# generic-ebpf/generic-ebpf

Measured on AMD Instinct MI355X. Metric: Mpkt/s device-resident (64-insn filter, 64B pkts); achieved HBM GB/s vs peak, higher is better.
Workload: dtype u64; 1 GPU; c4; desc=64-insn classify + array-map lookup, 64 B packets, packets_total=67108864, packets_per_gpu=67108864, packet_bytes=64, prog_slots=553, dprog_entries=122, variant=0, exec=compiled, kernel_layout=staged64, parallelism=dp1, launch=eager, faulted_packets=0

## Files before the change

### generic-ebpf_amd/csrc/asm/gen_interp.py

```python
#!/usr/bin/env python3
import os
import re
import sys

NREG = 11
_NT = int(os.environ.get("EBPF_ASM_NT", "3"))
ST_POLICY = " nt" if _NT & 1 else ""
LD_POLICY = " nt" if _NT & 2 else ""
PROBE_POLICY = ""
for _v, _n in (("EBPF_ASM_STPOL", "ST_POLICY"), ("EBPF_ASM_LDPOL", "LD_POLICY"),
               ("EBPF_ASM_PROBEPOL", "PROBE_POLICY")):
    if os.environ.get(_v):
        _p = os.environ[_v].replace("+", " ")
        globals()[_n] = "" if _p == "none" else " " + _p
PKT0 = 22
V_PKT = 38
V_LEN = 40
V_T = 41
V_STK = 42
V_L16 = 43
V_IDX = 43
V_RES = 44
H = [46, 47, 48, 49, 50, 51]
R = list(range(52, 63))
# ... 1914 lines not shown
          ".Llk_known:",
          "v_mov_b32 %s, v4" % v(H[0]), "v_mov_b32 %s, v5" % v(H[1]),
          "s_mov_b32 %s, 4" % s(S_T0), "s_mov_b32 %s, 0" % s(S_T1)] + call(".Lr_check")
    key = v(H[2])
    L += ["v_mov_b32 %s, 0" % key]
    for b in range(4):
        L += ["flat_load_ubyte %s, %s offset:%d" % (v(H[3]), vp(H[0]), b),
              "s_waitcnt vmcnt(0) lgkmcnt(0)",
              "v_lshl_or_b32 %s, %s, %d, %s" % (key, v(H[3]), 8 * b, key)]
    L += ["s_mov_b32 %s, 0" % s(S_T2),
          ".Llk_map:",
          "s_cmp_ge_u32 %s, %s" % (s(S_T2), s(S_NMAPS)),
          "s_cbranch_scc1 .Llk_done",
          "s_lshl_b32 %s, %s, 5" % (s(S_T3), s(S_T2)),
          "s_load_dwordx8 s[%d:%d], %s, %s" % (S_REC, S_REC + 7, sp(S_MAPS), s(S_T3)),
          "s_waitcnt lgkmcnt(0)",
          "v_cmp_eq_u64_e64 %s, v[2:3], s[64:65]" % sp(S_JUNK),
          "v_cmp_gt_u32_e64 vcc, s69, %s" % key,
          "s_and_b64 vcc, vcc, %s" % sp(S_JUNK),
          "v_mov_b32 %s, s68" % v(H[3]),
          "v_mad_u64_u32 %s, %s, %s, %s, s[66:67]" % (vp(H[4]), sp(S_JUNK), key, v(H[3])),
          "v_cndmask_b32 v0, v0, %s, vcc" % v(H[4]),
          "v_cndmask_b32 v1, v1, %s, vcc" % v(H[5]),
          "s_add_u32 %s, %s, 1" % (s(S_T2), s(S_T2)),
          "s_branch .Llk_map",
          ".Llk_done:",
          mode_test(MODE_JIT),
          "s_cbranch_scc1 .Llk_jit"] + dispatch(12) + [
          ".Llk_jit:",
          "s_add_u32 %s, %s, s12" % (s(S_JUNK), s(S_CB)),
          "s_addc_u32 %s, %s, 0" % (s(S_JUNK + 1), s(S_CB + 1)),
          "s_setpc_b64 %s" % sp(S_JUNK)] + [
          ".Llk_sched:"] + goto(".Lr_schedule")
    L += hlookup_routine()
    L += update_routine()
    L += hdelete_routine()
    L += vstore_routine()
    L += [".Lr_ovlfix:"] + ovl_fix("L", (H[2], H[3])) + ["s_setpc_b64 %s" % sp(S_LINK)]
    L += [".Lr_prefetch:",
          "s_mov_b64 exec, -1",
          "s_cmp_ge_u32 %s, %s" % (s(S_T0), s(S_NGROUPS)),
          "s_cbranch_scc1 .Lpf_ret",
          "s_lshl_b32 s66, %s, 6" % s(S_T0),
          "s_sub_u32 s66, %s, s66" % s(S_COUNT),
          "s_mov_b32 s64, %s" % s(S_T0),
          "s_mov_b32 s65, 0",
          "s_lshl_b64 s[64:65], s[64:65], 12",
          "s_add_u32 s64, s64, %s" % s(S_DATA),
          "s_addc_u32 s65, s65, %s" % s(S_DATA + 1),
          "s_mov_b32 s67, %s" % s(S_PKTLDS)] + dma_lane_offsets(v(H[4]), v(H[5]))
    for qq in range(4):
        L += ["s_sub_i32 s68, s66, %d" % (16 * qq),
              "s_max_i32 s68, s68, 0",
              "s_min_u32 s68, s68, 16",
              "s_lshl_b32 s68, s68, 6",
              "v_cmp_gt_u32_e64 vcc, s68, %s" % v(H[4]),
              "s_mov_b64 exec, vcc",
              "s_mov_b32 m0, s67",
              "s_nop 0",
              "global_load_lds_dwordx4 %s, s[64:65]%s" % (v(H[4]), LD_POLICY)]
        if qq < 3:
            L += ["s_add_u32 s64, s64, 1024", "s_addc_u32 s65, s65, 0",
                  "s_add_u32 s67, s67, 1024"]
    L += [".Lpf_ret:",
          "s_setpc_b64 %s" % sp(S_LINK)]
    return L


def kernel(name, staged, jit=False):
    k = "K%s%s" % ("s" if staged else "g", "j" if jit else "")
    L = [".globl %s" % name, ".p2align 8", ".type %s,@function" % name, "%s:" % name]
    if name == "ebpf_jit_s64" and phased() and SLOTS == 16:
        L += [".globl ebpf_jit_s64w", ".type ebpf_jit_s64w,@function", "ebpf_jit_s64w:"]
    L += ["v_readfirstlane_b32 %s, v0" % s(S_WAVE),
          "s_lshr_b32 %s, %s, 6" % (s(S_WAVE), s(S_WAVE)),
          "s_load_dwordx16 s[%d:%d], %s" % (S_PROG, S_PROG + 15, karg_regs(
              ("prog", S_PROG), ("maps", S_MAPS), ("data", S_DATA), ("offsets", S_OFFS),
              ("off_base", S_OFFBASE), ("ret", S_RET), ("faults", S_FAULTS), ("hist", S_HIST))),
          "s_load_dwordx8 s[%d:%d], %s" % (S_COUNT, S_COUNT + 7, karg_regs(
              ("count", S_COUNT), ("stride", S_STRIDE), ("start", S_START), ("nmaps", S_NMAPS),
              ("nentries", S_NENT), ("stack_stride", S_STKSTRIDE), ("lds_stack_base", S_LDSBASE))),
          "s_load_dword %s, %s" % (s(S_GSTRIDE), karg("total_waves")),
          "s_load_dword %s, %s" % (s(S_PKTLDS), karg("lds_pkt_base")),
          "s_mov_b64 %s, src_shared_base" % sp(S_SHARED),
          "v_mov_b32 v%d, 0x00010203" % V_SEL,
          "s_getpc_b64 %s" % sp(S_CB),
          ".L%s_pc:" % k,
          "s_add_u32 %s, %s, .Lcb-.L%s_pc" % (s(S_CB), s(S_CB), k),
          "s_addc_u32 %s, %s, 0" % (s(S_CB + 1), s(S_CB + 1)),
          "v_mbcnt_lo_u32_b32 %s, -1, 0" % v(H[0]),
          "v_mbcnt_hi_u32_b32 %s, -1, %s" % (v(H[0]), v(H[0])),
          "v_lshlrev_b32 v%d, 4, %s" % (V_L16, v(H[0])),
          "s_mov_b32 %s, -1" % s(S_PREVG),
          "s_waitcnt lgkmcnt(0)",
          "s_mov_b32 %s, %d" % (s(S_MODE), (staged << MODE_STAGED) | (jit << MODE_JIT)),
          "s_load_dword %s, %s" % (s(S_T3), karg("vflags"))] + (
          ["s_load_dword %s, %s" % (s(S_WPHASE), karg("wphase")) if staged else
           "s_mov_b32 %s, 0" % s(S_WPHASE),
           "s_mov_b32 %s, 0" % s(S_PEND)] if phased() else []) + [
          "s_waitcnt lgkmcnt(0)",
          "s_bitcmp1_b32 %s, %d" % (s(S_T3), VF_OVERLAY),
          "s_cbranch_scc0 .L%s_noovl" % k,
          mode_set(MODE_OVERLAY),
          ".L%s_noovl:" % k,
          "s_bitcmp1_b32 %s, %d" % (s(S_T3), VF_EXTENTS),
          "s_cbranch_scc0 .L%s_noext" % k,
          mode_set(MODE_EXTENTS),
          ".L%s_noext:" % k]
    if staged:
        L += ["s_bitcmp1_b32 %s, %d" % (s(S_T3), VF_KEEP),
              "s_cbranch_scc0 .L%s_nokeep" % k,
              mode_set(MODE_KEEP),
              ".L%s_nokeep:" % k]
    if not staged:
        L += ["s_bitcmp1_b32 %s, %d" % (s(S_PKTLDS), PKTLDS_HDRSTAGE),
              "s_cbranch_scc0 .L%s_nogs" % k,
              mode_set(MODE_HDRSTAGE),
              ".L%s_nogs:" % k,
              "s_bitcmp1_b32 %s, %d" % (s(S_PKTLDS), PKTLDS_HDRKEEP),
              "s_cbranch_scc0 .L%s_nohl" % k,
              mode_set(MODE_KEEP),
              ".L%s_nohl:" % k,
              "s_and_b32 %s, %s, 0x%x" % (s(S_PKTLDS), s(S_PKTLDS), (1 << PKTLDS_HDRKEEP) - 1)]
    L += ["s_branch .Lprologue"]
    return L


def lane_index(dst):
    if STAGED_IMAGE:
        return ["v_lshrrev_b32 %s, 4, v%d" % (v(dst), V_L16)]
    return ["v_mbcnt_lo_u32_b32 %s, -1, 0" % v(dst), "v_mbcnt_hi_u32_b32 %s, -1, %s" % (v(dst), v(dst))]


def lane_pkt_index(dst):
    if STAGED_IMAGE:
        return ["v_lshrrev_b32 %s, 4, v%d" % (v(dst), V_L16),
                "v_lshl_add_u32 %s, %s, 6, %s" % (v(dst), s(S_GROUP), v(dst))]
    return ["v_mov_b32 %s, v%d" % (v(dst), V_IDX)]


def pkt_setup(idx, tag):
    return ["s_mov_b64 %s, exec" % sp(S_MASK),
            "s_cmp_eq_u64 %s, 0" % sp(S_OFFS),
            "s_cbranch_scc0 .Lps_offsets_%s" % tag,
            "v_mov_b32 %s, %s" % (v(H[1]), s(S_STRIDE)),
            "v_mad_u64_u32 v[%d:%d], %s, v%d, %s, %s" % (V_PKT, V_PKT + 1, sp(S_JUNK), idx,
                                                         v(H[1]), sp(S_DATA)),
            "v_mov_b32 v%d, %s" % (V_LEN, s(S_STRIDE)),
            "s_branch .Lps_stage_%s" % tag,
            ".Lps_offsets_%s:" % tag,
            mode_test(MODE_EXTENTS),
            "s_cselect_b32 %s, 16, 8" % s(S_JUNK),
            "v_mov_b32 %s, %s" % (v(H[1]), s(S_JUNK)),
            "v_mad_u64_u32 %s, %s, v%d, %s, %s" % (vp(H[4]), sp(S_JUNK), idx, v(H[1]), sp(S_OFFS)),
            "global_load_dwordx2 %s, %s, off offset:8" % (vp(R[0]), vp(H[4])),
            "global_load_dwordx2 %s, %s, off" % (vp(H[4]), vp(H[4])),
            "s_waitcnt vmcnt(0)",
            "v_sub_co_u32 v%d, vcc, %s, %s" % (V_LEN, v(R[0]), v(H[4])),
            "v_subb_co_u32 %s, vcc, %s, %s, vcc" % (v(R[1]), v(R[1]), v(H[5])),
            "v_cmp_ne_u32_e32 vcc, 0, %s" % v(R[1]),
            "v_cndmask_b32 v%d, v%d, 0, vcc" % (V_LEN, V_LEN),
            "v_mov_b32 %s, %s" % (v(R[2]), s(S_OFFBASE + 1)),
            "v_sub_co_u32 %s, vcc, %s, %s" % (v(H[4]), v(H[4]), s(S_OFFBASE)),
            "v_subb_co_u32 %s, vcc, %s, %s, vcc" % (v(H[5]), v(H[5]), v(R[2])),
            "v_lshl_add_u64 v[%d:%d], %s, 0, %s" % (V_PKT, V_PKT + 1, vp(H[4]), sp(S_DATA)),
            ] + [
            ".Lps_stage_%s:" % tag,
            mode_test(MODE_HDRSTAGE),
            "s_cbranch_scc0 .Lps_done_%s" % tag,
            "v_cmp_lt_u32_e64 vcc, 63, v%d" % V_LEN,
            "s_and_b64 exec, %s, vcc" % sp(S_MASK),
            "s_cbranch_execz .Lps_done_%s" % tag] + [
            "global_load_dwordx4 v[%d:%d], v[%d:%d], off offset:%d" % (PKT0 + 4 * q, PKT0 + 4 * q + 3,
                                                                       V_PKT, V_PKT + 1, 16 * q)
            for q in range(4)] + [
            "s_waitcnt vmcnt(0)",
            mode_test(MODE_KEEP),
            "s_cbranch_scc0 .Lps_done_%s" % tag,
            "v_mbcnt_lo_u32_b32 %s, -1, 0" % v(H[1]),
            "v_mbcnt_hi_u32_b32 %s, -1, %s" % (v(H[1]), v(H[1])),
            "v_lshl_add_u32 %s, %s, 2, %s" % (v(H[1]), v(H[1]), s(S_PKTLDS))] + lds_pkt_dwords(v(H[1])) + [
            ".Lps_done_%s:" % tag,
            "s_mov_b64 exec, %s" % sp(S_MASK)]
# ... 91 lines not shown
                sk = ".Lph_%s%d_%d_%s" % ("r" if ragged else "f", half, j, tag)
                out += ["s_bitcmp1_b32 %s, %d" % (P, j), "s_cbranch_scc0 %s" % sk]
                if not ragged:
                    if own:
                        out += ["s_cmp_ge_u32 %s, %d" % (s(S_T3), i),
                                "s_cselect_b64 s[66:67], s[60:61], s[64:65]"]
                    out.append("global_store_dwordx2 %s, v[%d:%d], s[%d:%d] offset:%d%s" % (
                        v(R[0]), V_RB + 2 * j, V_RB + 2 * j + 1, 66 if own else 62,
                        67 if own else 63, 512 * i, ST_POLICY))
                else:
                    if own:
                        out += ["s_cmp_ge_u32 %s, %d" % (s(S_T3), i),
                                "s_cselect_b32 %s, %s, %s" % (s(S_BYTES), s(S_T1), s(S_T2))]
                    else:
                        out.append("s_mov_b32 %s, %s" % (s(S_BYTES), s(S_T0)))
                    out += ["s_add_u32 %s, %s, %d" % (s(S_BYTES), s(S_BYTES), i),
                            "s_lshl_b32 s66, %s, 6" % s(S_BYTES),
                            "s_sub_u32 s66, %s, s66" % s(S_COUNT),
                            "v_cmp_gt_u32_e64 vcc, s66, %s" % v(R[1]),
                            "s_mov_b64 exec, vcc",
                            "s_lshl_b32 s66, %s, 9" % s(S_BYTES),
                            "s_lshr_b32 s67, %s, 23" % s(S_BYTES),
                            "s_add_u32 s66, s66, %s" % s(S_RET),
                            "s_addc_u32 s67, s67, %s" % s(S_RET + 1),
                            "global_store_dwordx2 %s, v[%d:%d], s[66:67]%s" % (
                                v(R[0]), V_RB + 2 * j, V_RB + 2 * j + 1, ST_POLICY),
                            "s_mov_b64 exec, -1"]
                out.append(sk + ":")
        return out

    for ragged in (False, True):
        if ragged:
            L += [".Lph_ragged_%s:" % tag,
                  "v_lshrrev_b32 %s, 4, v%d" % (v(R[1]), V_L16)]
        if len(halves) > 1:
            L += ["s_bitcmp1_b32 %s, 31" % P,
                  "s_cbranch_scc1 .Lph_%sh1_%s" % ("r" if ragged else "f", tag)]
        L += slots_of(0, ragged) + ["s_branch .Lph_done_%s" % tag]
        if len(halves) > 1:
            L += [".Lph_%sh1_%s:" % ("r" if ragged else "f", tag)] + slots_of(1, ragged) + [
                  "s_branch .Lph_done_%s" % tag]
    L += [".Lph_done_%s:" % tag,
          "s_and_b32 %s, %s, 0x80000000" % (P, P),
          "s_branch .Lsp_none_%s" % tag,
          ".Lph_off_%s:" % tag]
    return L


def store_prev_results(tag, final):
    L = store_phased(tag, final) if phased() else []
    L += ["s_cmp_eq_u32 %s, -1" % s(S_PREVG),
         "s_cbranch_scc1 .Lsp_none_%s" % tag]
    if not final and RETK > 1:
        L += ["s_and_b32 %s, %s, %s" % (s(S_T0), s(S_PREVG), s(S_KMASK)),
              "s_cmp_lg_u32 %s, %s" % (s(S_T0), s(S_KMASK)),
              "s_cbranch_scc1 .Lsp_none_%s" % tag]
    L += ["s_mov_b64 exec, -1",
          "s_andn2_b32 %s, %s, %s" % (s(S_T0), s(S_PREVG), s(S_KMASK)) if RETK > 1 else
          "s_mov_b32 %s, %s" % (s(S_T0), s(S_PREVG)),
          ] + (["v_lshrrev_b32 %s, 4, v%d" % (v(R[1]), V_L16),
                "v_lshl_add_u32 %s, %s, 6, %s" % (v(R[1]), s(S_T0), v(R[1]))] if STAGED_IMAGE else
               ["v_mov_b32 %s, v%d" % (v(R[1]), V_IDX)]) + [
          "v_lshlrev_b32 %s, 3, %s" % (v(R[0]), v(R[1]))]
    for k in range(RETK):
        if k:
            L += ["s_cmp_lt_u32 %s, %d" % (s(S_KMASK), k),
                  "s_cbranch_scc1 .Lsp_none_%s" % tag,
                  "v_add_u32 %s, 64, %s" % (v(R[1]), v(R[1]))]
        L += ["v_cmp_gt_u32_e64 vcc, %s, %s" % (s(S_COUNT), v(R[1])),
              "s_mov_b64 exec, vcc",
              "global_store_dwordx2 %s, v[%d:%d], %s offset:%d%s" % (
                  v(R[0]), V_RB + 2 * k, V_RB + 2 * k + 1, sp(S_RET), 512 * k, ST_POLICY)]
    L.append(".Lsp_none_%s:" % tag)
    return L


def next_group(dst):
    return ["s_and_b32 %s, %s, %s" % (s(dst), s(S_GROUP), s(S_KMASK)),
            "s_cmp_eq_u32 %s, %s" % (s(dst), s(S_KMASK)),
            "s_cselect_b32 %s, %s, 1" % (s(dst), s(S_GSTRIDE)),
            "s_add_u32 %s, %s, %s" % (s(dst), s(dst), s(S_GROUP))]


def common_group_code():
    L = [".Lcb:",
         "ebpf_cb:",
         ".Lprologue:"]
    L += ["s_lshl_b32 %s, %s, 6" % (s(S_T0), s(S_WAVE)),
          "v_add_u32 %s, %s, %s" % (v(H[1]), s(S_T0), v(H[0])),
          "v_mul_lo_u32 %s, %s, %s" % (v(H[4]), v(H[1]), s(S_STKSTRIDE)),
          "v_add_u32 v%d, %s, %s" % (V_STK, s(S_LDSBASE), v(H[4]))]
    L += ["v_lshlrev_b32 %s, 2, %s" % (v(H[2]), v(H[1])),
          "v_mov_b32 %s, 0" % v(H[3]),
          "ds_write_b32 %s, %s" % (v(H[2]), v(H[3]))]
    L += ["v_lshlrev_b32 %s, 2, %s" % (v(H[4]), v(H[1])),
          "s_mov_b32 %s, 0" % s(S_T2),
          ".Lmc_loop:",
          "s_cmp_ge_u32 %s, %s" % (s(S_T2), s(S_NMAPS)),
          "s_cbranch_scc1 .Lmc_done",
          "s_lshl_b32 %s, %s, 5" % (s(S_T3), s(S_T2)),
          "s_load_dwordx8 s[%d:%d], %s, %s" % (S_REC, S_REC + 7, sp(S_MAPS), s(S_T3)),
          "s_waitcnt lgkmcnt(0)",
          "s_add_u32 %s, %s, 1" % (s(S_T2), s(S_T2)),
          "s_cmp_eq_u32 s70, -1",
          "s_cbranch_scc1 .Lmc_loop",
          "s_mul_i32 %s, s68, s69" % s(S_T1),
          "s_mov_b32 %s, 0" % s(S_T0),
          ".Lmc_chunk:",
          "s_cmp_ge_u32 %s, %s" % (s(S_T0), s(S_T1)),
          "s_cbranch_scc1 .Lmc_zero",
          "v_add_u32 %s, %s, %s" % (v(H[5]), s(S_T0), v(H[4])),
          "v_cmp_gt_u32_e64 vcc, %s, %s" % (s(S_T1), v(H[5])),
          "s_mov_b64 exec, vcc",
          "global_load_dword %s, %s, s[66:67]" % (v(H[3]), v(H[5])),
          "s_waitcnt vmcnt(0)",
          "v_add_u32 %s, s70, %s" % (v(H[5]), v(H[5])),
          "ds_write_b32 %s, %s" % (v(H[5]), v(H[3])),
          "s_mov_b64 exec, -1",
          "s_add_u32 %s, %s, 1024" % (s(S_T0), s(S_T0)),
          "s_branch .Lmc_chunk",
          ".Lmc_zero:",
          "s_bitcmp1_b32 s71, 29",
          "s_cbranch_scc0 .Lmc_loop",
          "s_and_b32 %s, s71, 0xffff" % s(S_T3),
          "v_mov_b32 %s, 0" % v(H[3]),
          "s_mov_b32 %s, 0" % s(S_T0),
          ".Lmc_zchunk:",
          "s_cmp_ge_u32 %s, %s" % (s(S_T0), s(S_T1)),
          "s_cbranch_scc1 .Lmc_loop",
          "v_add_u32 %s, %s, %s" % (v(H[5]), s(S_T0), v(H[4])),
          "v_cmp_gt_u32_e64 vcc, %s, %s" % (s(S_T1), v(H[5])),
          "s_mov_b64 exec, vcc",
          "v_add_u32 %s, %s, %s" % (v(H[5]), s(S_T3), v(H[5])),
          "ds_write_b32 %s, %s" % (v(H[5]), v(H[3])),
          "s_mov_b64 exec, -1",
          "s_add_u32 %s, %s, 1024" % (s(S_T0), s(S_T0)),
          "s_branch .Lmc_zchunk",
          ".Lmc_done:",
          "s_waitcnt lgkmcnt(0)",
          "s_barrier"]
    L += ["s_add_u32 %s, %s, 63" % (s(S_NGROUPS), s(S_COUNT)),
          "s_lshr_b32 %s, %s, 6" % (s(S_NGROUPS), s(S_NGROUPS)),
          "s_lshl_b32 %s, s2, 2" % s(S_GROUP),
          "s_add_u32 %s, %s, %s" % (s(S_GROUP), s(S_GROUP), s(S_WAVE)),
          "s_lshr_b32 %s, %s, %d" % (s(S_T1), s(S_GSTRIDE), WAVES_SB_SHIFT),
          "s_and_b32 %s, %s, 0xffff" % (s(S_GSTRIDE), s(S_GSTRIDE)),
          "s_lshl_b32 %s, 1, %s" % (s(S_KMASK), s(S_T1)),
          "s_sub_u32 %s, %s, 1" % (s(S_KMASK), s(S_KMASK)),
          "s_lshl_b32 %s, %s, %s" % (s(S_GROUP), s(S_GROUP), s(S_T1)),
          ] + [
          "s_lshl_b32 %s, %s, %s" % (s(S_GSTRIDE), s(S_GSTRIDE), s(S_T1)),
          "s_sub_u32 %s, %s, %s" % (s(S_GSTRIDE), s(S_GSTRIDE), s(S_KMASK)),
          "s_lshl_b32 %s, %s, 12" % (s(S_T0), s(S_WAVE)),
          "s_add_u32 %s, %s, %s" % (s(S_PKTLDS), s(S_PKTLDS), s(S_T0)),
          mode_test(MODE_STAGED),
          "s_cbranch_scc0 .Lgroup_check",
          "s_mov_b32 %s, %s" % (s(S_T0), s(S_GROUP))] + call(".Lr_prefetch") + [
          "s_branch .Lgroup_check"]
    L += [".Lgroup_done:"]
    L += slot_commit() + next_group(S_T0) + [
          "s_and_b32 %s, %s, 0x%x" % (s(S_BYTES), s(S_MODE), 1 << MODE_KEEP | 1 << MODE_STAGED),
          "s_cmp_eq_u32 %s, 0x4001" % s(S_BYTES),
          "s_cbranch_scc0 .Lgd_nokeep"] + call(".Lr_prefetch") + [
          ".Lgd_nokeep:",
          "s_mov_b32 %s, %s" % (s(S_GROUP), s(S_T0)),
          ".Lgroup_check:",
          "s_mov_b64 exec, -1",
          "s_cmp_lt_u32 %s, %s" % (s(S_GROUP), s(S_NGROUPS)),
          "s_cbranch_scc0 .Lfinish",
          ] + (
          ["s_cmp_eq_u32 %s, 0" % s(S_WPHASE),
           "s_cbranch_scc1 .Lgc_noclock",
           "s_memrealtime s[%d:%d]" % (S_CLOCK, S_CLOCK + 1),
           ".Lgc_noclock:"] if phased() else []) + lane_index(H[0]) + [
          "v_lshl_add_u32 v%d, %s, 6, %s" % (V_GIDX, s(S_GROUP), v(H[0])),
          "v_cmp_gt_u32_e64 %s, %s, v%d" % (sp(S_ALIVE), s(S_COUNT), V_GIDX),
          ] + [
          mode_test(MODE_STAGED),
          "s_cbranch_scc0 .Lgs_general",
          "s_waitcnt vmcnt(0)",
          "v_and_b32 %s, 0x300, v%d" % (v(H[1]), V_L16),
          "v_mad_u32_u24 %s, %s, 3, v%d" % (v(H[1]), v(H[1]), V_L16),
          "v_add_u32 %s, %s, %s" % (v(H[1]), s(S_PKTLDS), v(H[1]))]
    for q in range(4):
        L.append("ds_read_b128 v[%d:%d], %s offset:%d" % (PKT0 + 4 * q, PKT0 + 4 * q + 3,
                                                          v(H[1]), 256 * q))
    L += ["s_waitcnt lgkmcnt(0)",
          mode_test(MODE_KEEP),
          "s_cbranch_scc0 .Lgs_pf_dma",
          "v_lshrrev_b32 %s, 2, v%d" % (v(H[1]), V_L16),
          "v_add_u32 %s, %s, %s" % (v(H[1]), s(S_PKTLDS), v(H[1]))] + lds_pkt_dwords(v(H[1])) + [
          "s_branch .Lgs_pf_done",
          ".Lgs_pf_dma:"] + next_group(S_T0) + [
          "s_lshr_b32 %s, %s, 6" % (s(S_BYTES), s(S_COUNT)),
          "s_cmp_lt_u32 %s, %s" % (s(S_T0), s(S_BYTES)),
          "s_cbranch_scc0 .Lgs_pf_slow",
          "s_lshr_b32 s65, %s, 20" % s(S_T0),
          "s_lshl_b32 s64, %s, 12" % s(S_T0),
          "s_add_u32 s64, s64, %s" % s(S_DATA),
          "s_addc_u32 s65, s65, %s" % s(S_DATA + 1),
          "s_mov_b64 exec, -1"] + dma_lane_offsets(v(H[4]), v(H[5])) + [
          "s_mov_b32 m0, %s" % s(S_PKTLDS),
          "s_nop 0"] + [
          "global_load_lds_dwordx4 %s, s[64:65] offset:%d%s" % (v(H[4]), 1024 * qq, LD_POLICY)
          for qq in range(4)] + [
          "s_branch .Lgs_pf_done",
          ".Lgs_pf_slow:"] + call(".Lr_prefetch") + [
          ".Lgs_pf_done:",
          mode_test(MODE_JIT),
          "s_cbranch_scc1 .Lgs_init",
          "s_mov_b64 exec, %s" % sp(S_ALIVE),
          "v_mov_b32 %s, 64" % v(H[1]),
          "v_mad_u64_u32 v[%d:%d], %s, v%d, %s, %s" % (V_PKT, V_PKT + 1, sp(S_JUNK), V_GIDX,
                                                       v(H[1]), sp(S_DATA)),
          "v_mov_b32 v%d, 64" % V_LEN,
          "s_branch .Lgs_init",
          ".Lgs_general:",
          "s_mov_b64 exec, %s" % sp(S_ALIVE)] + pkt_setup(V_GIDX, "g") + [
          ".Lgs_init:"] + store_prev_results("g", False) + [
          "s_mov_b32 %s, %s" % (s(S_PREVG), s(S_GROUP))] + ([] if STAGED_IMAGE else [
          "s_mov_b64 exec, -1",
          "v_mov_b32 v%d, v%d" % (V_IDX, V_GIDX)]) + [
          "s_mov_b64 exec, %s" % sp(S_ALIVE),
          "s_cmp_eq_u64 %s, 0" % sp(S_FAULTS),
          "s_cbranch_scc1 .Lgs_nofz",
          ] + lane_pkt_index(R[9]) + [
          "v_mov_b32 %s, 0" % v(R[8]),
          "global_store_byte %s, %s, %s" % (v(R[9]), v(R[8]), sp(S_FAULTS)),
          ".Lgs_nofz:",
          mode_test(MODE_JIT),
          "s_cbranch_scc0 .Lgs_interp"] + goto("ebpf_jit_area+%d" % JIT_ENTRY_OFF) + [
          ".Lgs_interp:"]
    for r in range(0, 20, 2):
        if r != 2:
            L.append("v_mov_b64 v[%d:%d], 0" % (r, r + 1))
    L += ["v_mov_b64 v[2:3], v[%d:%d]" % (V_PKT, V_PKT + 1),
          "v_add_u32 v20, %s, v%d" % (s(S_STKSTRIDE), V_STK),
          "v_mov_b32 v21, %s" % s(S_SHARED + 1),
          "s_lshl_b32 %s, %s, 5" % (s(S_T0), s(S_START)),
          "v_mov_b32 v%d, %s" % (V_T, s(S_T0))] + goto(".Lr_schedule")
    HR = HIST_REPLICA_BYTES
    L += [".Lfinish:"] + store_prev_results("f", True)
    L += [".Lfinish_body:",
          "s_mov_b64 exec, -1",
          "s_waitcnt vmcnt(0) lgkmcnt(0)",
          "s_barrier"]
    L += lane_index(H[0]) + [
          "s_lshl_b32 %s, %s, 6" % (s(S_T0), s(S_WAVE)),
          "v_add_u32 %s, %s, %s" % (v(H[1]), s(S_T0), v(H[0])),
          "s_mov_b32 %s, 0" % s(S_T2),
          ".Lfd_loop:",
          "s_cmp_ge_u32 %s, %s" % (s(S_T2), s(S_NMAPS)),
          "s_cbranch_scc1 .Lfd_done",
          "s_lshl_b32 %s, %s, 5" % (s(S_T3), s(S_T2)),
          "s_load_dwordx8 s[%d:%d], %s, %s" % (S_REC, S_REC + 7, sp(S_MAPS), s(S_T3)),
          "s_waitcnt lgkmcnt(0)",
          "s_add_u32 %s, %s, 1" % (s(S_T2), s(S_T2)),
          "s_bitcmp1_b32 s71, 29",
          "s_cbranch_scc0 .Lfd_loop",
          "s_mul_i32 %s, s68, s69" % s(S_T1),
          "s_add_u32 %s, %s, 63" % (s(S_BYTES), s(S_T1)),
          "s_and_b32 %s, %s, -64" % (s(S_BYTES), s(S_BYTES)),
          "s_add_u32 s66, s66, %s" % s(S_BYTES),
          "s_addc_u32 s67, s67, 0",
          "s_and_b32 %s, s71, 0xffff" % s(S_T3),
          "s_bitcmp1_b32 s71, 28",
          "s_cselect_b32 %s, 3, 2" % s(S_CODE),
          "v_lshlrev_b32 %s, %s, %s" % (v(H[2]), s(S_CODE), v(H[1])),
          "s_lshl_b32 %s, 256, %s" % (s(S_BYTES), s(S_CODE)),
          ".Lfd_word:",
          "v_cmp_gt_u32_e64 vcc, %s, %s" % (s(S_T1), v(H[2])),
          "s_and_saveexec_b64 %s, vcc" % sp(S_MASK),
          "s_cbranch_execz .Lfd_next",
          "v_add_u32 %s, %s, %s" % (v(H[3]), s(S_T3), v(H[2])),
          "v_mov_b32 %s, 0" % v(R[3]),
          "s_cmp_eq_u32 %s, 3" % s(S_CODE),
          "s_cbranch_scc0 .Lfd_r4",
          "ds_read_b64 %s, %s" % (vp(R[2]), v(H[3])),
          "s_branch .Lfd_r",
          ".Lfd_r4:",
          "ds_read_b32 %s, %s" % (v(R[2]), v(H[3])),
          ".Lfd_r:",
          "s_waitcnt lgkmcnt(0)",
          "v_cmp_ne_u64_e64 vcc, 0, %s" % vp(R[2]),
          "s_and_b64 exec, exec, vcc",
          "s_cbranch_execz .Lfd_next",
          "v_mov_b32 %s, %s" % (v(R[0]), v(H[2])),
          "s_cmp_eq_u32 %s, 3" % s(S_CODE),
          "s_cbranch_scc0 .Lfd_w4",
          "global_atomic_add_x2 %s, %s, s[66:67]" % (v(R[0]), vp(R[2])),
          "s_branch .Lfd_next",
          ".Lfd_w4:",
          "global_atomic_add %s, %s, s[66:67]" % (v(R[0]), v(R[2])),
          ".Lfd_next:",
          "s_mov_b64 exec, %s" % sp(S_MASK),
          "v_add_u32 %s, %s, %s" % (v(H[2]), s(S_BYTES), v(H[2])),
          "v_cmp_gt_u32_e64 vcc, %s, %s" % (s(S_T1), v(H[2])),
          "s_and_b64 vcc, vcc, exec",
          "s_cbranch_scc1 .Lfd_word",
          "s_mov_b64 exec, -1",
          "s_branch .Lfd_loop",
          ".Lfd_done:",
          "s_mov_b64 exec, -1",
          "s_cmp_eq_u64 %s, 0" % sp(S_HIST),
          "s_cbranch_scc1 .Lfin_end",
          ] + lane_index(H[0]) + [
          "s_lshl_b32 %s, %s, 6" % (s(S_T0), s(S_WAVE)),
          "v_add_u32 %s, %s, %s" % (v(H[1]), s(S_T0), v(H[0])),
          "v_lshlrev_b32 %s, 2, %s" % (v(H[2]), v(H[1])),
          "ds_read_b32 %s, %s" % (v(H[3]), v(H[2])),
          "s_load_dwordx2 %s, %s" % (sp(S_REC), karg("hist_rows")),
          "s_load_dwordx4 s[68:71], %s" % karg("hist_user", "hist_flags", "nwg"),
          "s_waitcnt lgkmcnt(0)",
          "s_cmp_eq_u64 %s, 0" % sp(S_REC),
          "s_cbranch_scc1 .Lfin_atomic",
          "s_and_b32 %s, s2, 7" % s(S_T1),
          "s_mul_i32 %s, %s, %d" % (s(S_T1), s(S_T1), HR),
          "v_lshlrev_b32 %s, 3, %s" % (v(R[0]), v(H[1])),
          "v_add_u32 %s, %s, %s" % (v(R[0]), s(S_T1), v(R[0])),
          "v_mov_b32 %s, %s" % (v(R[2]), v(H[3])),
          "v_mov_b32 %s, 0" % v(R[3]),
          "v_cmp_ne_u32_e64 vcc, 0, %s" % v(H[3]),
          "s_and_saveexec_b64 %s, vcc" % sp(S_SAVE),
          "s_cbranch_execz .Lfin_noadd",
          "global_atomic_add_x2 %s, %s, %s" % (v(R[0]), vp(R[2]), sp(S_REC)),
          ".Lfin_noadd:",
          "s_mov_b64 exec, -1",
          "s_waitcnt vmcnt(0)",
          "s_barrier",
          "s_cmp_eq_u32 %s, 0" % s(S_WAVE),
          "s_cbranch_scc0 .Lfin_flag",
          "s_mov_b64 exec, 1",
          "s_and_b32 %s, s2, 7" % s(S_T1),
          "s_lshl_b32 %s, %s, 6" % (s(S_T0), s(S_T1)),
          "s_add_u32 %s, %s, %d" % (s(S_T0), s(S_T0), HIST_TICKET_OFF),
          "v_mov_b32 %s, %s" % (v(R[4]), s(S_T0)),
          "v_mov_b32 %s, 1" % v(R[5]),
          "global_atomic_add %s, %s, %s, %s sc0" % (v(R[6]), v(R[4]), v(R[5]), sp(S_REC)),
          "s_sub_u32 %s, s71, 1" % s(S_T3),
          "s_sub_u32 %s, %s, %s" % (s(S_T3), s(S_T3), s(S_T1)),
          "s_lshr_b32 %s, %s, 3" % (s(S_T3), s(S_T3)),
          "s_waitcnt vmcnt(0)",
          "v_readfirstlane_b32 %s, %s" % (s(S_T2), v(R[6])),
          "s_cmp_eq_u32 %s, %s" % (s(S_T2), s(S_T3)),
          "s_cselect_b32 %s, 1, 0" % s(S_T2),
          "s_cbranch_scc0 .Lfin_setflag",
          "v_mov_b32 %s, 0" % v(R[10]),
          "global_atomic_swap %s, %s, %s, %s sc0" % (v(R[8]), v(R[4]), v(R[10]), sp(S_REC)),
          "v_mov_b32 %s, %d" % (v(R[9]), HIST_TICKET_OFF + 64 * HIST_REPLICAS),
          "global_atomic_add %s, %s, %s, %s sc0" % (v(R[6]), v(R[9]), v(R[5]), sp(S_REC)),
          "s_min_u32 %s, s71, %d" % (s(S_T3), HIST_REPLICAS),
          "s_sub_u32 %s, %s, 1" % (s(S_T3), s(S_T3)),
          "s_waitcnt vmcnt(0)",
          "v_readfirstlane_b32 %s, %s" % (s(S_T2), v(R[6])),
          "s_cmp_eq_u32 %s, %s" % (s(S_T2), s(S_T3)),
          "s_cselect_b32 %s, 1, 0" % s(S_T2),
          ".Lfin_setflag:",
          "v_mov_b32 %s, %s" % (v(R[7]), s(S_T2)),
          "v_mov_b32 %s, 0" % v(R[8]),
          "ds_write_b32 %s, %s" % (v(R[8]), v(R[7])),
          "s_mov_b64 exec, -1",
          "s_waitcnt lgkmcnt(0)",
          ".Lfin_flag:",
          "s_barrier",
          "v_mov_b32 %s, 0" % v(R[8]),
          "ds_read_b32 %s, %s" % (v(R[7]), v(R[8])),
          "s_waitcnt lgkmcnt(0)",
          "v_readfirstlane_b32 %s, %s" % (s(S_T2), v(R[7])),
          "s_cmp_eq_u32 %s, 0" % s(S_T2),
          "s_cbranch_scc1 .Lfin_end",
          "v_lshlrev_b32 %s, 3, %s" % (v(R[0]), v(H[1])),
          "v_mov_b32 v24, 0",
          "v_mov_b32 v25, 0"]
    for r in range(HIST_REPLICAS):
        L += ["v_add_u32 v%d, %d, %s" % (16 + r, r * HR, v(R[0])),
              "global_atomic_swap_x2 v[%d:%d], v%d, v[24:25], %s sc0" % (2 * r, 2 * r + 1, 16 + r,
                                                                       sp(S_REC))]
    L += ["s_waitcnt vmcnt(0)"]
    for r in range(1, HIST_REPLICAS):
        L += ["v_lshl_add_u64 v[0:1], v[%d:%d], 0, v[0:1]" % (2 * r, 2 * r + 1)]
    L += ["s_bitcmp1_b32 s70, %d" % HIST_STORE,
          "s_cbranch_scc0 .Lfin_add",
          "global_store_dwordx2 %s, v[0:1], s[68:69]" % v(R[0]),
          "s_branch .Lfin_faults",
          ".Lfin_add:",
          "global_atomic_add_x2 %s, v[0:1], s[68:69]" % v(R[0]),
          ".Lfin_faults:",
          "s_cmp_eq_u32 %s, 0" % s(S_WAVE),
          "s_cbranch_scc0 .Lfin_end",
          "s_mov_b64 exec, 1",
          "v_mov_b32 v16, 2048",
          "global_atomic_swap_x2 v[2:3], v16, v[24:25], %s sc0" % sp(S_REC),
          "v_mov_b32 v17, %d" % (HIST_TICKET_OFF + 64 * HIST_REPLICAS),
          "global_atomic_swap v18, v17, v24, %s sc0" % sp(S_REC),
          "s_waitcnt vmcnt(0)",
          "s_bitcmp1_b32 s70, %d" % HIST_STORE,
          "s_cbranch_scc0 .Lfin_fadd",
          "global_store_dwordx2 v16, v[2:3], s[68:69]",
          "s_branch .Lfin_end",
          ".Lfin_fadd:",
          "global_atomic_add_x2 v16, v[2:3], s[68:69]",
          "s_branch .Lfin_end",
          ".Lfin_atomic:",
          "v_cmp_ne_u32_e64 vcc, 0, %s" % v(H[3]),
          "s_and_saveexec_b64 %s, vcc" % sp(S_SAVE),
          "v_lshlrev_b32 %s, 3, %s" % (v(R[0]), v(H[1])),
          "v_mov_b32 %s, %s" % (v(R[2]), v(H[3])),
          "v_mov_b32 %s, 0" % v(R[3]),
          "global_atomic_add_x2 %s, %s, %s" % (v(R[0]), vp(R[2]), sp(S_HIST)),
          ".Lfin_end:",
          "s_waitcnt vmcnt(0)",
          "s_endpgm"]
    return L


def link_kernel():
    return [".globl ebpf_asm_link", ".p2align 8", ".type ebpf_asm_link,@function",
            "ebpf_asm_link:",
            "s_load_dwordx2 s[4:5], %s" % karg("entries", table=LINK_ARGS),
            "s_load_dword s6, %s" % karg("count", table=LINK_ARGS),
            "s_getpc_b64 s[8:9]",
            ".Llink_base:",
            "s_add_u32 s10, s8, .Lhandler_table-.Llink_base",
            "s_addc_u32 s11, s9, 0",
            "v_lshl_add_u32 v1, s2, 6, v0",
            "s_waitcnt lgkmcnt(0)",
            "v_cmp_gt_u32_e64 vcc, s6, v1",
            "s_and_b64 exec, exec, vcc",
            "s_cbranch_execz .Llink_end",
            "v_mov_b32 v2, 32",
            "v_mad_u64_u32 v[2:3], s[12:13], v1, v2, s[4:5]",
            "global_load_dword v4, v[2:3], off",
            "s_waitcnt vmcnt(0)",
            "v_mov_b32 v6, 4",
            "v_mad_u64_u32 v[6:7], s[12:13], v4, v6, s[10:11]",
            "global_load_dword v8, v[6:7], off",
            "s_waitcnt vmcnt(0)",
            "v_ashrrev_i32 v9, 31, v8",
            "v_lshl_add_u64 v[10:11], v[8:9], 0, s[8:9]",
            "global_store_dwordx2 v[2:3], v[10:11], off",
            ".Llink_end:",
            "s_waitcnt vmcnt(0)",
            "s_endpgm"]


def kd(name, lds, vgprs, sgprs, kernarg, wgsize):
    return [".rodata", ".p2align 6", ".amdhsa_kernel %s" % name,
            ".amdhsa_group_segment_fixed_size %d" % lds,
            ".amdhsa_private_segment_fixed_size 0",
            ".amdhsa_kernarg_size %d" % kernarg,
            ".amdhsa_user_sgpr_count 2",
            ".amdhsa_user_sgpr_kernarg_segment_ptr 1",
            ".amdhsa_system_sgpr_workgroup_id_x 1",
            ".amdhsa_system_vgpr_workitem_id 0",
            ".amdhsa_next_free_vgpr %d" % vgprs,
            ".amdhsa_next_free_sgpr %d" % sgprs,
            ".amdhsa_accum_offset %d" % vgprs,
            ".amdhsa_reserve_vcc 1",
            ".amdhsa_reserve_xnack_mask 0",
            ".amdhsa_ieee_mode 0",
            ".amdhsa_dx10_clamp 0",
            ".end_amdhsa_kernel", ".text"]


def metadata(kernels):
    out = [".amdgpu_metadata", "---", "amdhsa.kernels:"]
    for name, kernarg, lds, vgprs, sgprs, wg in kernels:
        out += ["  - .args:",
                "      - .offset: 0",
                "        .size: %d" % kernarg,
                "        .value_kind: by_value",
                "    .group_segment_fixed_size: %d" % lds,
                "    .kernarg_segment_align: 8",
                "    .kernarg_segment_size: %d" % kernarg,
                "    .max_flat_workgroup_size: %d" % wg,
                "    .name: %s" % name,
                "    .private_segment_fixed_size: 0",
                "    .sgpr_count: %d" % sgprs,
                "    .symbol: %s.kd" % name,
                "    .vgpr_count: %d" % vgprs,
                "    .wavefront_size: 64"]
    out += ["amdhsa.target: amdgcn-amd-amdhsa--gfx950:xnack-", "amdhsa.version:", "  - 1", "  - 2",
            "...", ".end_amdgpu_metadata"]
    return out


JIT_AREA_BYTES = 512 * 1024
JIT_ENTRY_OFF = 16
ENTRY_SGPR_RE = None


def entry_reads(lines):
    import re
    global ENTRY_SGPR_RE
    if ENTRY_SGPR_RE is None:
# ... 294 lines not shown
```

Measured before the change: 84820 Mpkt/s.

## Pipeline map-cache prologue loads and overlap prologue/finish latencies

Hoists the vflags/wphase kernel-argument loads into the first scalar load batch so only one lgkmcnt wait is needed. Rewrites the map-to-LDS copy loop to issue up to 16 global loads into distinct VGPRs before a single drain, instead of waiting on each load. The LDS barrier now comes after the staged prefetch is issued, so the two overlap. The finish path drops a vmcnt wait and issues the fault-counter swaps before the histogram swaps so their latencies overlap. It uses v0-v31 as temporaries in the prologue and adds nop padding, which risks register clobbering and ordering bugs.

```diff
diff --git a/generic-ebpf_amd/csrc/asm/gen_interp.py b/generic-ebpf_amd/csrc/asm/gen_interp.py
--- a/generic-ebpf_amd/csrc/asm/gen_interp.py
+++ b/generic-ebpf_amd/csrc/asm/gen_interp.py
@@ -2020,6 +2020,8 @@
               ("nentries", S_NENT), ("stack_stride", S_STKSTRIDE), ("lds_stack_base", S_LDSBASE))),
           "s_load_dword %s, %s" % (s(S_GSTRIDE), karg("total_waves")),
           "s_load_dword %s, %s" % (s(S_PKTLDS), karg("lds_pkt_base")),
+          "s_load_dword %s, %s" % (s(S_T3), karg("vflags"))] + (
+          ["s_load_dword %s, %s" % (s(S_WPHASE), karg("wphase"))] if phased() and staged else []) + [
           "s_mov_b64 %s, src_shared_base" % sp(S_SHARED),
           "v_mov_b32 v%d, 0x00010203" % V_SEL,
           "s_getpc_b64 %s" % sp(S_CB),
@@ -2032,11 +2034,9 @@
           "s_mov_b32 %s, -1" % s(S_PREVG),
           "s_waitcnt lgkmcnt(0)",
           "s_mov_b32 %s, %d" % (s(S_MODE), (staged << MODE_STAGED) | (jit << MODE_JIT)),
-          "s_load_dword %s, %s" % (s(S_T3), karg("vflags"))] + (
-          ["s_load_dword %s, %s" % (s(S_WPHASE), karg("wphase")) if staged else
-           "s_mov_b32 %s, 0" % s(S_WPHASE),
-           "s_mov_b32 %s, 0" % s(S_PEND)] if phased() else []) + [
-          "s_waitcnt lgkmcnt(0)",
+          ] + (
+          ([] if staged else ["s_mov_b32 %s, 0" % s(S_WPHASE)]) +
+          ["s_mov_b32 %s, 0" % s(S_PEND)] if phased() else []) + [
           "s_bitcmp1_b32 %s, %d" % (s(S_T3), VF_OVERLAY),
           "s_cbranch_scc0 .L%s_noovl" % k,
           mode_set(MODE_OVERLAY),
@@ -2294,63 +2294,13 @@
             "s_add_u32 %s, %s, %s" % (s(dst), s(dst), s(S_GROUP))]
 
 
+MC_SLOTS = 16
+
+
 def common_group_code():
     L = [".Lcb:",
          "ebpf_cb:",
          ".Lprologue:"]
-    L += ["s_lshl_b32 %s, %s, 6" % (s(S_T0), s(S_WAVE)),
-          "v_add_u32 %s, %s, %s" % (v(H[1]), s(S_T0), v(H[0])),
-          "v_mul_lo_u32 %s, %s, %s" % (v(H[4]), v(H[1]), s(S_STKSTRIDE)),
-          "v_add_u32 v%d, %s, %s" % (V_STK, s(S_LDSBASE), v(H[4]))]
-    L += ["v_lshlrev_b32 %s, 2, %s" % (v(H[2]), v(H[1])),
-          "v_mov_b32 %s, 0" % v(H[3]),
-          "ds_write_b32 %s, %s" % (v(H[2]), v(H[3]))]
-    L += ["v_lshlrev_b32 %s, 2, %s" % (v(H[4]), v(H[1])),
-          "s_mov_b32 %s, 0" % s(S_T2),
-          ".Lmc_loop:",
-          "s_cmp_ge_u32 %s, %s" % (s(S_T2), s(S_NMAPS)),
-          "s_cbranch_scc1 .Lmc_done",
-          "s_lshl_b32 %s, %s, 5" % (s(S_T3), s(S_T2)),
-          "s_load_dwordx8 s[%d:%d], %s, %s" % (S_REC, S_REC + 7, sp(S_MAPS), s(S_T3)),
-          "s_waitcnt lgkmcnt(0)",
-          "s_add_u32 %s, %s, 1" % (s(S_T2), s(S_T2)),
-          "s_cmp_eq_u32 s70, -1",
-          "s_cbranch_scc1 .Lmc_loop",
-          "s_mul_i32 %s, s68, s69" % s(S_T1),
-          "s_mov_b32 %s, 0" % s(S_T0),
-          ".Lmc_chunk:",
-          "s_cmp_ge_u32 %s, %s" % (s(S_T0), s(S_T1)),
-          "s_cbranch_scc1 .Lmc_zero",
-          "v_add_u32 %s, %s, %s" % (v(H[5]), s(S_T0), v(H[4])),
-          "v_cmp_gt_u32_e64 vcc, %s, %s" % (s(S_T1), v(H[5])),
-          "s_mov_b64 exec, vcc",
-          "global_load_dword %s, %s, s[66:67]" % (v(H[3]), v(H[5])),
-          "s_waitcnt vmcnt(0)",
-          "v_add_u32 %s, s70, %s" % (v(H[5]), v(H[5])),
-          "ds_write_b32 %s, %s" % (v(H[5]), v(H[3])),
-          "s_mov_b64 exec, -1",
-          "s_add_u32 %s, %s, 1024" % (s(S_T0), s(S_T0)),
-          "s_branch .Lmc_chunk",
-          ".Lmc_zero:",
-          "s_bitcmp1_b32 s71, 29",
-          "s_cbranch_scc0 .Lmc_loop",
-          "s_and_b32 %s, s71, 0xffff" % s(S_T3),
-          "v_mov_b32 %s, 0" % v(H[3]),
-          "s_mov_b32 %s, 0" % s(S_T0),
-          ".Lmc_zchunk:",
-          "s_cmp_ge_u32 %s, %s" % (s(S_T0), s(S_T1)),
-          "s_cbranch_scc1 .Lmc_loop",
-          "v_add_u32 %s, %s, %s" % (v(H[5]), s(S_T0), v(H[4])),
-          "v_cmp_gt_u32_e64 vcc, %s, %s" % (s(S_T1), v(H[5])),
-          "s_mov_b64 exec, vcc",
-          "v_add_u32 %s, %s, %s" % (v(H[5]), s(S_T3), v(H[5])),
-          "ds_write_b32 %s, %s" % (v(H[5]), v(H[3])),
-          "s_mov_b64 exec, -1",
-          "s_add_u32 %s, %s, 1024" % (s(S_T0), s(S_T0)),
-          "s_branch .Lmc_zchunk",
-          ".Lmc_done:",
-          "s_waitcnt lgkmcnt(0)",
-          "s_barrier"]
     L += ["s_add_u32 %s, %s, 63" % (s(S_NGROUPS), s(S_COUNT)),
           "s_lshr_b32 %s, %s, 6" % (s(S_NGROUPS), s(S_NGROUPS)),
           "s_lshl_b32 %s, s2, 2" % s(S_GROUP),
@@ -2365,10 +2315,85 @@
           "s_sub_u32 %s, %s, %s" % (s(S_GSTRIDE), s(S_GSTRIDE), s(S_KMASK)),
           "s_lshl_b32 %s, %s, 12" % (s(S_T0), s(S_WAVE)),
           "s_add_u32 %s, %s, %s" % (s(S_PKTLDS), s(S_PKTLDS), s(S_T0)),
+          "s_mov_b64 exec, -1"]
+    L += ["s_lshl_b32 %s, %s, 6" % (s(S_T0), s(S_WAVE)),
+          "v_add_u32 %s, %s, %s" % (v(H[1]), s(S_T0), v(H[0])),
+          "v_mul_lo_u32 %s, %s, %s" % (v(H[4]), v(H[1]), s(S_STKSTRIDE)),
+          "v_add_u32 v%d, %s, %s" % (V_STK, s(S_LDSBASE), v(H[4]))]
+    L += ["v_lshlrev_b32 %s, 2, %s" % (v(H[2]), v(H[1])),
+          "v_mov_b32 %s, 0" % v(H[3]),
+          "ds_write_b32 %s, %s" % (v(H[2]), v(H[3]))]
+    NS = MC_SLOTS
+    L += ["v_lshlrev_b32 %s, 2, %s" % (v(H[4]), v(H[1])),
+          "s_mov_b32 %s, 0" % s(S_T2),
+          "s_mov_b32 %s, 0" % s(S_T0),
+          "s_mov_b32 %s, 0" % s(S_T1),
+          ".Lmc_s0:",
+          "s_mov_b32 %s, 0" % s(S_CODE)]
+    for k in range(NS):
+        L += [".Lmc_s%d:" % k if k else ".Lmc_s0b:",
+              "s_cmp_lt_u32 %s, %s" % (s(S_T0), s(S_T1)),
+              "s_cbranch_scc1 .Lmc_i%d" % k,
+              ".Lmc_a%d:" % k,
+              "s_cmp_ge_u32 %s, %s" % (s(S_T2), s(S_NMAPS)),
+              "s_cbranch_scc1 .Lmc_w%d" % k,
+              "s_lshl_b32 %s, %s, 5" % (s(S_T3), s(S_T2)),
+              "s_load_dwordx8 s[%d:%d], %s, %s" % (S_REC, S_REC + 7, sp(S_MAPS), s(S_T3)),
+              "s_add_u32 %s, %s, 1" % (s(S_T2), s(S_T2)),
+              "s_waitcnt lgkmcnt(0)",
+              "s_cmp_eq_u32 s70, -1",
+              "s_cbranch_scc1 .Lmc_a%d" % k,
+              "s_mul_i32 %s, s68, s69" % s(S_T1),
+              "s_mov_b32 %s, 0" % s(S_T0),
+              "s_bitcmp1_b32 s71, 29",
+              "s_cbranch_scc0 .Lmc_s%s" % (k if k else "0b")] + call(".Lmc_zero") + [
+              "s_branch .Lmc_s%s" % (k if k else "0b"),
+              ".Lmc_i%d:" % k,
+              "v_add_u32 %s, %s, %s" % (v(H[5]), s(S_T0), v(H[4])),
+              "v_cmp_gt_u32_e64 vcc, %s, %s" % (s(S_T1), v(H[5])),
+              "s_mov_b64 exec, vcc",
+              "global_load_dword v%d, %s, s[66:67]" % (k, v(H[5])),
+              "s_mov_b64 exec, -1",
+              "v_add_u32 %s, s70, %s" % (v(H[5]), v(H[5])),
+              "v_cndmask_b32 v%d, -1, %s, vcc" % (NS + k, v(H[5])),
+              "s_add_u32 %s, %s, 1024" % (s(S_T0), s(S_T0))]
+    L += ["s_mov_b32 %s, 1" % s(S_CODE)]
+    for k in range(NS, 0, -1):
+        L += [".Lmc_w%d:" % k,
+              "s_waitcnt vmcnt(0)",
+              "s_mov_b64 exec, -1",
+              "v_cmp_ne_u32_e64 vcc, -1, v%d" % (NS + k - 1),
+              "s_mov_b64 exec, vcc",
+              "ds_write_b32 v%d, v%d" % (NS + k - 1, k - 1)]
+    L += [".Lmc_w0:",
+          "s_mov_b64 exec, -1",
+          "s_cmp_eq_u32 %s, 1" % s(S_CODE),
+          "s_cbranch_scc1 .Lmc_s0",
           mode_test(MODE_STAGED),
-          "s_cbranch_scc0 .Lgroup_check",
+          "s_cbranch_scc0 .Lpro_nopf",
           "s_mov_b32 %s, %s" % (s(S_T0), s(S_GROUP))] + call(".Lr_prefetch") + [
-          "s_branch .Lgroup_check"]
+          ".Lpro_nopf:",
+          "s_waitcnt lgkmcnt(0)",
+          "s_barrier",
+          "s_branch .Lgroup_check",
+          ".Lmc_zero:",
+          "s_and_b32 %s, s71, 0xffff" % s(S_T3),
+          "v_mov_b32 %s, 0" % v(H[3]),
+          "s_mov_b32 %s, 0" % s(S_BYTES),
+          ".Lmc_zchunk:",
+          "s_cmp_ge_u32 %s, %s" % (s(S_BYTES), s(S_T1)),
+          "s_cbranch_scc1 .Lmc_zret",
+          "v_add_u32 %s, %s, %s" % (v(H[5]), s(S_BYTES), v(H[4])),
+          "v_cmp_gt_u32_e64 vcc, %s, %s" % (s(S_T1), v(H[5])),
+          "s_mov_b64 exec, vcc",
+          "v_add_u32 %s, %s, %s" % (v(H[5]), s(S_T3), v(H[5])),
+          "ds_write_b32 %s, %s" % (v(H[5]), v(H[3])),
+          "s_mov_b64 exec, -1",
+          "s_add_u32 %s, %s, 1024" % (s(S_BYTES), s(S_BYTES)),
+          "s_branch .Lmc_zchunk",
+          ".Lmc_zret:",
+          "s_setpc_b64 %s" % sp(S_LINK)]
+    L += ["s_nop 0"] * 5
     L += [".Lgroup_done:"]
     L += slot_commit() + next_group(S_T0) + [
           "s_and_b32 %s, %s, 0x%x" % (s(S_BYTES), s(S_MODE), 1 << MODE_KEEP | 1 << MODE_STAGED),
@@ -2455,7 +2480,7 @@
     L += [".Lfinish:"] + store_prev_results("f", True)
     L += [".Lfinish_body:",
           "s_mov_b64 exec, -1",
-          "s_waitcnt vmcnt(0) lgkmcnt(0)",
+          "s_waitcnt lgkmcnt(0)",
           "s_barrier"]
     L += lane_index(H[0]) + [
           "s_lshl_b32 %s, %s, 6" % (s(S_T0), s(S_WAVE)),
@@ -2583,7 +2608,16 @@
           "s_cbranch_scc1 .Lfin_end",
           "v_lshlrev_b32 %s, 3, %s" % (v(R[0]), v(H[1])),
           "v_mov_b32 v24, 0",
-          "v_mov_b32 v25, 0"]
+          "v_mov_b32 v25, 0",
+          "s_cmp_eq_u32 %s, 0" % s(S_WAVE),
+          "s_cbranch_scc0 .Lfin_swaps",
+          "s_mov_b64 exec, 1",
+          "v_mov_b32 v28, 2048",
+          "global_atomic_swap_x2 v[26:27], v28, v[24:25], %s sc0" % sp(S_REC),
+          "v_mov_b32 v29, %d" % (HIST_TICKET_OFF + 64 * HIST_REPLICAS),
+          "global_atomic_swap v30, v29, v24, %s sc0" % sp(S_REC),
+          "s_mov_b64 exec, -1",
+          ".Lfin_swaps:"]
     for r in range(HIST_REPLICAS):
         L += ["v_add_u32 v%d, %d, %s" % (16 + r, r * HR, v(R[0])),
               "global_atomic_swap_x2 v[%d:%d], v%d, v[24:25], %s sc0" % (2 * r, 2 * r + 1, 16 + r,
@@ -2601,17 +2635,12 @@
           "s_cmp_eq_u32 %s, 0" % s(S_WAVE),
           "s_cbranch_scc0 .Lfin_end",
           "s_mov_b64 exec, 1",
-          "v_mov_b32 v16, 2048",
-          "global_atomic_swap_x2 v[2:3], v16, v[24:25], %s sc0" % sp(S_REC),
-          "v_mov_b32 v17, %d" % (HIST_TICKET_OFF + 64 * HIST_REPLICAS),
-          "global_atomic_swap v18, v17, v24, %s sc0" % sp(S_REC),
-          "s_waitcnt vmcnt(0)",
           "s_bitcmp1_b32 s70, %d" % HIST_STORE,
           "s_cbranch_scc0 .Lfin_fadd",
-          "global_store_dwordx2 v16, v[2:3], s[68:69]",
+          "global_store_dwordx2 v28, v[26:27], s[68:69]",
           "s_branch .Lfin_end",
           ".Lfin_fadd:",
-          "global_atomic_add_x2 v16, v[2:3], s[68:69]",
+          "global_atomic_add_x2 v28, v[26:27], s[68:69]",
           "s_branch .Lfin_end",
           ".Lfin_atomic:",
           "v_cmp_ne_u32_e64 vcc, 0, %s" % v(H[3]),
@@ -2623,6 +2652,7 @@
           ".Lfin_end:",
           "s_waitcnt vmcnt(0)",
           "s_endpgm"]
+    L += ["s_nop 0"] * 13
     return L
 
 
```

New measurement: 84890 Mpkt/s (median of 6 runs). About the same (+0.1%).
